# evolbioinfo/pastml

Hardware: AMD Instinct MI355X
Metric: ACR nodes*states*chars/sec (full marginal pass: P(t) + bottom-up + top-down + posteriors) (higher is better)
Workload: dtype f64; 1 GPU; BASELINE config 4 shard: balanced tree, 1048576 tips (2097151 nodes), k=64 states, F81, 32 characters per GPU (32 in total), marginal (BU+TD+posteriors); tips=1048576, nodes=2097151, states=64, chars_per_gpu=32, chars_total=32, substitution_model=F81, collective=local

## Files before the change

pastml_amd/csrc/pml_kernels_f81.h:

```cpp
#pragma once
#include "pml_device.h"
#include "pml_schedule.h"

typedef unsigned char pml_jt;

struct PmlTree {
    int N;
    int n_roots;
    const int* parent;
    const int* first_child;
    const int* n_children;
    const double* dist;
    const int* post_rank;
    const unsigned char* kind;
};

struct PmlCols {
    int k, ks, W;
    int no_wide_lean;
    const u64* masks;
    const u64* masks_init;
    const double* pi;
    const double* active;
};
// ... 1523 lines not shown
template <int G, int R>
__device__ __forceinline__ void bu_f81_super_issue(const LaneCtx<G, R>& L, const SuperRegs& s, SuperLoads<R>& ld) {
#pragma unroll
    for (int j = 0; j < 2; ++j) {
        const UnitRegs u = super_child<G>(s, j, L.g);
        f81_gather_issue<G, R>(L, u, ld.c[j].cl, ld.c[j].tl);
        ld.c[j].own = L.mask[(unsigned)u.n];
    }
    ld.e = L.E[s.fc + (L.g & 1)];
    ld.own = L.mask[(unsigned)s.n];
}

template <int R>
__device__ __forceinline__ void super_loads_arrived(SuperLoads<R>& ld) {
#pragma unroll
    for (int j = 0; j < 2; ++j)
        asm volatile("" : "+v"(ld.c[j].cl.e), "+v"(ld.c[j].cl.mask), "+v"(ld.c[j].tl.e), "+v"(ld.c[j].tl.s),
                          "+v"(ld.c[j].tl.mask), "+v"(ld.c[j].own));
    asm volatile("" : "+v"(ld.e), "+v"(ld.own));
}

template <int G, int R>
__device__ __forceinline__ bool bu_f81_super_unit(const LaneCtx<G, R>& L, const PmlTree& t, const PmlCols& c,
                                                  const PmlState& st, const SuperRegs& s, SuperLoads<R>& ld) {
    super_loads_arrived<R>(ld);
    const u64 kbits = state_bits(c.k);
    bool ones = c.k == G * R;
#pragma unroll
    for (int j = 0; j < 2; ++j) {
        f81_gather_finish<G, R>(L, ld.c[j].cl, ld.c[j].tl);
        ones = ones && (ld.c[j].own & kbits) == kbits && ld.c[j].cl.mask == kbits;
    }
    const bool full = __all(ones);
    BuResult<R> res[2];
#pragma unroll
    for (int j = 0; j < 2; ++j) {
        const UnitRegs u = super_child<G>(s, j, L.g);
        const bool ok = full ? bu_f81_marg_body<G, R, false, true, true>(L, t, c, st, u, ld.c[j], &res[j], false)
                             : bu_f81_marg_body<G, R, false, false, true>(L, t, c, st, u, ld.c[j], &res[j], false);
        if (!ok) return false;
    }
    BuLoads<R> top;
    top.cl.e = ld.e;
    top.cl.s = (L.g & 1) ? res[1].s : res[0].s;
    top.cl.be = (L.g & 1) ? res[1].e : res[0].e;
    top.cl.mask = kbits;
    top.tl.e = top.tl.s = top.tl.a = 0.0;
    top.tl.mask = 0ull;
    top.own = ld.own;
#pragma unroll
    for (int r = 0; r < R; ++r) {
        top.v0[r] = res[0].v[r];
        top.v1[r] = res[1].v[r];
    }
    return bu_f81_marg_body<G, R, true, false>(L, t, c, st, super_own(s), top);
}

template <int G, int R>
__device__ __forceinline__ void bu_f81_super_seq(const LaneCtx<G, R>& L, const PmlTree& t, const PmlCols& c,
                                                 const PmlState& st, const SuperRegs& s) {
    bu_f81_unit_seq<G, R, false>(L, t, c, st, super_child<G>(s, 0, L.g));
    bu_f81_unit_seq<G, R, false>(L, t, c, st, super_child<G>(s, 1, L.g));
    __threadfence();
    bu_f81_unit_seq<G, R, false>(L, t, c, st, super_own(s));
}

template <int G, int R>
__global__ void __launch_bounds__(PML_BLOCK) __attribute__((amdgpu_waves_per_eu(2, 2)))
bu_f81_super_kernel(PmlTree t, PmlCols c, PmlState st, const PmlUnit* __restrict__ units, int n_level) {
    constexpr int UW = 64 / G;
    const int wave = threadIdx.x >> 6;
    const int sub = (threadIdx.x & 63) / G;
    LaneCtx<G, R> L;
    lane_ctx_init<G, R>(L, t, c, st);
    const int stride = gridDim.x * PML_WAVES_PER_BLOCK * UW;
    int idx = (blockIdx.x * PML_WAVES_PER_BLOCK + wave) * UW + sub;
    int base = idx - sub;
    SuperRegs ua = load_super(units, idx < n_level ? idx : 0);
    SuperRegs ub = load_super(units, idx + stride < n_level ? idx + stride : 0);
    SuperLoads<R> la, lb;
    bu_f81_super_issue<G, R>(L, ua, la);
    while (base < n_level) {
        {
            const int i2 = idx + 2 * stride;
            const SuperRegs un = load_super(units, i2 < n_level ? i2 : 0);
            bu_f81_super_issue<G, R>(L, ub, lb);
            if (idx < n_level) {
                if (!bu_f81_super_unit<G, R>(L, t, c, st, ua, la)) bu_f81_super_seq<G, R>(L, t, c, st, ua);
            }
            ua = un;
            idx += stride;
            base += stride;
        }
        if (base >= n_level) break;
        {
            const int i2 = idx + 2 * stride;
            const SuperRegs un = load_super(units, i2 < n_level ? i2 : 0);
            bu_f81_super_issue<G, R>(L, ua, la);
            if (idx < n_level) {
                if (!bu_f81_super_unit<G, R>(L, t, c, st, ub, lb)) bu_f81_super_seq<G, R>(L, t, c, st, ub);
            }
            ub = un;
            idx += stride;
            base += stride;
        }
    }
}

template <int G, int R>
__device__ __forceinline__ void f81_finish_child(const LaneCtx<G, R>& L, const PmlCols& c, const double (&prod)[R],
                                                 i64 pe, int ch, double e, double s_child, i64 bec,
                                                 const double (&v)[R], bool full_mask, const double (&mb)[R],
                                                 double (&tdc)[R], i64& xe, double (&lh)[R], double& lsum, i64& le,
                                                 int slot = -1) {
    const double a = (1.0 - e) * s_child;
    double x[R];
#pragma unroll
    for (int r = 0; r < R; ++r) {
        const double cn = fmax(a + e * v[r], 0x1p-1022);
        x[r] = prod[r] * rcp1(cn);
    }
    xe = pe - bec;
    const double b = (1.0 - e) * pi_dot<G, R>(L, x);
#pragma unroll
    for (int r = 0; r < R; ++r) tdc[r] = b + e * x[r];
    double lhs = 0.0;
    if (full_mask) {
#pragma unroll
        for (int r = 0; r < R; ++r) {
            lh[r] = v[r] * tdc[r] * L.pi_r[r];
            lhs += lh[r];
        }
    } else {
#pragma unroll
        for (int r = 0; r < R; ++r) {
            lh[r] = v[r] * tdc[r] * (L.pi_r[r] * mb[r]);
            lhs += lh[r];
        }
    }
    lhs = group_sum<G>(lhs);
    const int lex = (lhs > 0.0 && !isinf(lhs)) ? exponent_of(lhs) : 0;
    const double inv = rcp1(lhs);
#pragma unroll
    for (int r = 0; r < R; ++r) {
        const double q = lh[r] * inv;
        lh[r] = fma(fma(-lhs, q, lh[r]), inv, q);
    }
    const bool staged = post_row<G, R>(L, c, slot, ch, lh);
    lsum = __builtin_ldexp(lhs, -lex);
    le = xe + bec + lex;
    post_scalars<G, R>(L, staged ? slot : -1, ch, lsum, le);
}

template <int G, int R>
__device__ __forceinline__ void f81_finish_tip_word(const LaneCtx<G, R>& L, const PmlCols& c, const double (&prod)[R],
                                                    i64 pe, double& P, bool& have_P, int tip, u64 word, double e,
                                                    double pis, int slot = -1) {
    if (__popcll(word) == 1) {
        if (!have_P) {
            P = pi_dot<G, R>(L, prod);
            have_P = true;
        }
        double oh[R];
        clean_word_to_vec<G, R>(L, c, word, oh);
        double pick = 0.0;
#pragma unroll
        for (int r = 0; r < R; ++r) pick = fma(oh[r], prod[r], pick);
        const double ps = group_sum<G>(pick);
        const double q = pis * ps;
        double c0 = (1.0 - e) * pis;
        const double c1 = c0 + e;
        if (!(c0 > 0.0)) c0 = 1.0;
        const double r1 = rcp1(c1);
        const double sx = (P - q) * rcp1(c0) + q * r1;
        const double tds = (1.0 - e) * sx + e * (ps * r1);
        const double lhs = tds * pis;
        const bool ok = lhs > 0.0 && !isinf(lhs);
        const int lex = ok ? exponent_of(lhs) : 0;
        if (!ok) {
#pragma unroll
            for (int r = 0; r < R; ++r) oh[r] = __builtin_nan("");
        }
        const bool staged = post_onehot<G, R>(L, c, slot, tip, (int)__builtin_ctzll(word), oh, ok);
        post_scalars<G, R>(L, staged ? slot : -1, tip, __builtin_ldexp(lhs, -lex), pe + lex);
    } else {
        double mt[R], tdt[R], pt[R], lt;
        clean_word_to_vec<G, R>(L, c, word, mt);
        i64 xt, et;
        f81_finish_child<G, R>(L, c, prod, pe, tip, e, pis, 0, mt, false, mt, tdt, xt, pt, lt, et, slot);
    }
}

template <int G, int R>
__device__ __forceinline__ void f81_finish_tip(const LaneCtx<G, R>& L, const PmlCols& c, const double (&prod)[R], i64 pe,
                                               double& P, bool& have_P, int tip, int slot = -1) {
    const double e = L.E[tip];
    const double pis = L.S[tip];
    if (c.W == 1) {
        f81_finish_tip_word<G, R>(L, c, prod, pe, P, have_P, tip, L.mask[(unsigned)tip] & state_bits(c.k), e, pis,
                                  slot);
    } else {
        double mt[R], tdt[R], pt[R], lt;
        node_mask_vec<G, R>(L, c, tip, mt);
        i64 xt, et;
        f81_finish_child<G, R>(L, c, prod, pe, tip, e, pis, 0, mt, false, mt, tdt, xt, pt, lt, et, slot);
    }
}

template <int G, int R>
__device__ __forceinline__ void td_f81_fast_children(const LaneCtx<G, R>& L, const PmlTree& t, const PmlCols& c,
                                                     const PmlState& st, const UnitRegs& u, const double (&prod)[R],
                                                     i64 pe, const ChildLane& cl, const TipLane& tl, double (&vn)[R]);

template <int G, int R>
__device__ __forceinline__ void td_f81_unit_fast(const LaneCtx<G, R>& L, const PmlTree& t, const PmlCols& c,
                                                 const PmlState& st, const UnitRegs& u) {
    const int p = u.n, fc = u.fc;
    double prod[R];
    i64 pe;
    f81_parent_prod<G, R>(L, c, p, prod, pe);
    ChildLane cl;
    TipLane tl;
    f81_gather_issue<G, R>(L, u, cl, tl);
    double vn[R];
    if (unit_code(u.packed, 0) == 1) node_load_vec<G, R>(L, c, L.bu, fc, vn);
    f81_gather_finish<G, R>(L, cl, tl);
    td_f81_fast_children<G, R>(L, t, c, st, u, prod, pe, cl, tl, vn);
}

template <int G, int R>
__device__ __forceinline__ void td_f81_fast_children(const LaneCtx<G, R>& L, const PmlTree& t, const PmlCols& c,
                                                     const PmlState& st, const UnitRegs& u, const double (&prod)[R],
                                                     i64 pe, const ChildLane& cl, const TipLane& tl, double (&vn)[R]) {
    constexpr int GC = Gather<G>::GC;
    const int fc = u.fc;
    const int nc = unit_nc(u.packed);
    double P = 0.0;
    bool have_P = false;
    for (int jx = 0; jx < nc; ++jx) {
        const int src = L.group_base + jx;
        const int ch = fc + jx;
        const int code = unit_code(u.packed, jx);
        const double e = __shfl(cl.e, src, 64);
        const u64 word = __shfl(cl.mask, src, 64);
        double v[R];
        if (code == 1) {
#pragma unroll
            for (int r = 0; r < R; ++r) v[r] = vn[r];
        }
        if (jx + 1 < nc && unit_code(u.packed, jx + 1) == 1) node_load_vec<G, R>(L, c, L.bu, ch + 1, vn);
        if (code == 0) {
            f81_finish_tip_word<G, R>(L, c, prod, pe, P, have_P, ch, word, e, __shfl(cl.s, src, 64));
            continue;
        }
        double mb[R], tdc[R], po[R], ls;
        const bool full = word == state_bits(c.k);
        if (!full) clean_word_to_vec<G, R>(L, c, word, mb);
        i64 xe, le;
        if (code == 1) {
            f81_finish_child<G, R>(L, c, prod, pe, ch, e, __shfl(cl.s, src, 64), __shfl(cl.be, src, 64), v, full, mb,
                                   tdc, xe, po, ls, le);
            if (st.td != nullptr) {
                node_store_vec<G, R>(L, c, L.td, ch, tdc);
                if (L.g == 0) L.te[ch] = xe;
            }
        } else {
            i64 bec;
            const int cfc = __shfl(u.cfc, L.group_base + jx * GC, 64);
            const int cnc = code - 1;
            f81_cherry_from_lanes<G, R>(L, c, cl, tl, jx, cnc, v, bec);
            const double s_child = __shfl(cl.s, src, 64);
            f81_finish_child<G, R>(L, c, prod, pe, ch, e, s_child, bec, v, full, mb, tdc, xe, po, ls, le);
            double prod2[R];
#pragma unroll
            for (int r = 0; r < R; ++r) prod2[r] = po[r] * (ls * L.ipi_r[r]);
            const i64 pe2 = le;
            double P2 = 0.0;
            bool have_P2 = false;
            for (int q = 0; q < cnc; ++q) {
                const int ts = L.group_base + jx * GC + q;
                f81_finish_tip_word<G, R>(L, c, prod2, pe2, P2, have_P2, cfc + q, __shfl(tl.mask, ts, 64),
                                          __shfl(tl.e, ts, 64), __shfl(tl.s, ts, 64));
            }
        }
    }
}

template <int G, int R, int SC0 = PML_SHAPE_ANY, int SC1 = PML_SHAPE_ANY>
__device__ __forceinline__ void td_f81_unit_lean(const LaneCtx<G, R>& L, const PmlTree& t, const PmlCols& c,
                                                 const PmlState& st, const UnitRegs& u) {
    constexpr bool ANY = SC0 == PML_SHAPE_ANY;
    const int p = u.n, fc = u.fc;
    const int nc = ANY ? unit_nc(u.packed) : (SC1 < 0 ? 1 : 2);
    const u64 kbits = state_bits(c.k);
    double po[R];
    node_load_vec<G, R>(L, c, L.post, p, po);
    const double ls = L.lhsum[p];
    const i64 pe = L.lhe[p];
    double ce[2], cs[2], vv[2][R];
    u64 cm[2];
    i64 cbe[2];
    double te[2][2], ts[2][2];
    u64 tm[2][2];
#pragma unroll
    for (int j = 0; j < 2; ++j) {
        const int ch = fc + (j < nc ? j : 0);
        const int code = j < nc ? (ANY ? unit_code(u.packed, j) : (j == 0 ? SC0 : SC1)) : 0;
        ce[j] = L.E[ch];
        cm[j] = L.mask[(unsigned)ch];
        cs[j] = L.S[ch];
        cbe[j] = code == 1 ? L.be[ch] : 0;
        if (code == 1) {
            node_load_vec<G, R>(L, c, L.bu, ch, vv[j]);
        } else {
#pragma unroll
            for (int r = 0; r < R; ++r) vv[j][r] = 0.0;
        }
        const int cfc = j == 0 ? u.cfc : u.cfc1;
#pragma unroll
        for (int q = 0; q < 2; ++q) {
            const bool has = code >= 2 && q < code - 1;
            const int tip = has ? cfc + q : ch;
            te[j][q] = L.E[tip];
            ts[j][q] = has ? L.S[tip] : 0.0;
            tm[j][q] = L.mask[(unsigned)tip];
        }
    }
    double prod[R];
#pragma unroll
    for (int r = 0; r < R; ++r) prod[r] = po[r] * (ls * L.ipi_r[r]);
    double P = 0.0;
    bool have_P = false;
#pragma unroll
    for (int j = 0; j < 2; ++j) {
        if (j < nc) {
            const int ch = fc + j;
            const int code = ANY ? unit_code(u.packed, j) : (j == 0 ? SC0 : SC1);
// ... 310 lines not shown
    const int p = u.n;

    double prod[R];
    i64 pe;
    f81_parent_prod<G, R>(L, c, p, prod, pe);
    double P = 0.0;
    bool have_P = false;
    const int fc = u.fc;
    int nc = unit_nc(u.packed);
    if (nc == 15) nc = t.n_children[p];
    for (int j = 0; j < nc; ++j) {
        const int ch = fc + j;
        const ChildDesc cd = unit_child<G>(t, u, j, ch);
        const int kd = cd.kind;
        const int slot = j < 2 ? j : -1;
        if (kd == PML_KIND_TIP) {
            f81_finish_tip<G, R>(L, c, prod, pe, P, have_P, ch, slot);
            continue;
        }
        const double e = L.E[ch];
        double mb[R], v[R], tdc[R], po[R], ls;
        node_mask_vec<G, R>(L, c, ch, mb);
        i64 xe, le;
        if (kd == PML_KIND_STORED) {
            node_load_vec<G, R>(L, c, L.bu, ch, v);
            f81_finish_child<G, R>(L, c, prod, pe, ch, e, L.S[ch], L.be[ch], v, false, mb, tdc, xe, po, ls, le, slot);
            if (st.td != nullptr) {
                node_store_vec<G, R>(L, c, L.td, ch, tdc);
                if (L.g == 0) L.te[ch] = xe;
            }
        } else {
            i64 bec;
            f81_cherry_vector<G, R>(L, t, c, st, ch, v, bec, false, cd.tips_known, cd.fc2, cd.nc2);
            const double s_child = L.S[ch];
            f81_finish_child<G, R>(L, c, prod, pe, ch, e, s_child, bec, v, false, mb, tdc, xe, po, ls, le, slot);
            double prod2[R];
#pragma unroll
            for (int r = 0; r < R; ++r) prod2[r] = po[r] * (ls * L.ipi_r[r]);
            const i64 pe2 = le;
            double P2 = 0.0;
            bool have_P2 = false;
            const int fc2 = cd.tips_known ? cd.fc2 : t.first_child[ch];
            const int nc2 = cd.tips_known ? cd.nc2 : t.n_children[ch];
            for (int q = 0; q < nc2; ++q)
                f81_finish_tip<G, R>(L, c, prod2, pe2, P2, have_P2, fc2 + q, (j < 2 && q < 2) ? 2 + 2 * j + q : -1);
        }
    }
}

struct TdStage {
    double* rows;
    double* sum;
    i64* exp;
    int* id;
    int* tid;
    int* tst;
};
__host__ __device__ __forceinline__ int td_stage_doubles(int uw, int ks, bool scalars) {
    return uw * 2 * ks + (scalars ? uw * 12 : 0) + uw * 5;
}

template <int G, int R>
__device__ __forceinline__ void td_stage_flush(const LaneCtx<G, R>& L, const PmlCols& c, const TdStage& S, bool tips) {
    typedef double dbl2 __attribute__((ext_vector_type(2)));
    constexpr int UW = 64 / G;
    wave_sync_lds();
    const int lane = threadIdx.x & 63;
    const int ppr = c.ks >> 1;
    for (int p = lane; p < UW * 2 * ppr; p += 64) {
        const int slot = p / ppr, piece = p - slot * ppr;
        const int node = S.id[slot];
        if (node >= 0) {
            const dbl2 v = *reinterpret_cast<const dbl2*>(S.rows + slot * c.ks + 2 * piece);
            __builtin_nontemporal_store(v, reinterpret_cast<dbl2*>(L.post + (size_t)(unsigned)node * c.ks + 2 * piece));
        }
    }
    for (int p = lane; tips && p < UW * 4 * ppr; p += 64) {
        const int slot = p / ppr, piece = p - slot * ppr;
        const int node = S.tid[slot];
        if (node >= 0) {
            const int s = S.tst[slot];
            dbl2 v;
            v.x = s == 2 * piece ? 1.0 : 0.0;
            v.y = s == 2 * piece + 1 ? 1.0 : 0.0;
            __builtin_nontemporal_store(v, reinterpret_cast<dbl2*>(L.post + (size_t)(unsigned)node * c.ks + 2 * piece));
        }
    }
    if (S.sum != nullptr) {
        for (int e = lane; e < UW * 6; e += 64) {
            const int u = e / 6, j = e - u * 6;
            if (j >= 2 && !tips) continue;
            const int node = j < 2 ? S.id[u * 2 + j] : S.tid[u * 4 + j - 2];
            if (node >= 0) {
                L.lhsum[node] = S.sum[e];
                L.lhe[node] = S.exp[e];
            }
        }
    }
    wave_sync_lds();
    for (int e = lane; e < UW * 2; e += 64) S.id[e] = -1;
    for (int e = lane; tips && e < UW * 4; e += 64) S.tid[e] = -1;
    wave_sync_lds();
}

template <int G, int R>
__global__ void __launch_bounds__(PML_BLOCK)
td_f81_kernel(PmlTree t, PmlCols c, PmlState st, const PmlUnit* __restrict__ units, int n_level, int stage) {
    extern __shared__ double td_stage[];
    constexpr int UW = 64 / G;
    const int wave = threadIdx.x >> 6;
    const int sub = (threadIdx.x & 63) / G;
    LaneCtx<G, R> L;
    lane_ctx_init<G, R>(L, t, c, st);
    TdStage S = {nullptr, nullptr, nullptr, nullptr, nullptr, nullptr};
    const bool staged = G <= PML_TD_STAGE_MAX_G && (stage & 1) && (c.ks & 1) == 0;
    if (staged) {
        const bool scalars = (stage & 2) != 0;
        double* base = td_stage + wave * td_stage_doubles(UW, c.ks, scalars);
        S.rows = base;
        base += UW * 2 * c.ks;
        if (scalars) {
            S.sum = base;
            S.exp = reinterpret_cast<i64*>(base + UW * 6);
            base += UW * 12;
        }
        S.id = reinterpret_cast<int*>(base);
        S.tid = S.id + UW * 2;
        S.tst = S.tid + UW * 4;
        L.srow = S.rows + sub * 2 * c.ks;
        L.sid = S.id + sub * 2;
        L.stid = S.tid + sub * 4;
        L.stst = S.tst + sub * 4;
        if (scalars) {
            L.ssum = S.sum + sub * 6;
            L.sexp = S.exp + sub * 6;
        }
        for (int e = threadIdx.x & 63; e < UW * 2; e += 64) S.id[e] = -1;
        for (int e = threadIdx.x & 63; e < UW * 4; e += 64) S.tid[e] = -1;
        wave_sync_lds();
    }
    const int stride = gridDim.x * PML_WAVES_PER_BLOCK * UW;
    int idx = (blockIdx.x * PML_WAVES_PER_BLOCK + wave) * UW + sub;
    UnitRegs cur = load_unit<G>(units, idx < n_level ? idx : 0, L.g);
    for (int base = idx - sub; base < n_level; base += stride) {
        const int nxt_idx = idx + stride;
        const UnitRegs nxt = load_unit<G>(units, nxt_idx < n_level ? nxt_idx : 0, L.g);
        if (idx < n_level) td_f81_unit<G, R, true>(L, t, c, st, cur);
        if (staged) td_stage_flush<G, R>(L, c, S, (stage & 4) != 0);
        cur = nxt;
        idx = nxt_idx;
    }
}

template <int G, int R>
__device__ __forceinline__ void td_f81_super_unit(const LaneCtx<G, R>& L, const PmlTree& t, const PmlCols& c,
                                                  const PmlState& st, const SuperRegs& s, int j) {
    const u64 kbits = state_bits(c.k);
    const int ch = s.fc + j;
    const UnitRegs u = super_child<G>(s, j, L.g);
    double prod[R];
    i64 pe;
    f81_parent_prod<G, R>(L, c, s.n, prod, pe);
    const double e = L.E[ch];
    const double s_child = L.S[ch];
    const i64 bec = L.be[ch];
    BuLoads<R> ld;
    ld.own = L.mask[(unsigned)ch];
    f81_gather_issue<G, R>(L, u, ld.cl, ld.tl);
    f81_gather_finish<G, R>(L, ld.cl, ld.tl);
    ld.own &= kbits;
    const bool all_ones = __all(c.k == G * R && ld.own == kbits && ld.cl.mask == kbits);
    BuResult<R> v;
    CherryKeep<R> ck;
    if (all_ones) bu_f81_marg_body<G, R, false, true, true>(L, t, c, st, u, ld, &v, false, true, &ck);
    else bu_f81_marg_body<G, R, false, false, true>(L, t, c, st, u, ld, &v, false, true, &ck);
    double prod2[R];
    i64 pe2;
    {
        double mb[R], tdc[R], po[R], ls;
        const bool full = ld.own == kbits;
        if (!full) clean_word_to_vec<G, R>(L, c, ld.own, mb);
        i64 xe;
        f81_finish_child<G, R>(L, c, prod, pe, ch, e, s_child, bec, v.v, full, mb, tdc, xe, po, ls, pe2);
        if (st.td != nullptr) {
            node_store_vec<G, R>(L, c, L.td, ch, tdc);
            if (L.g == 0) L.te[ch] = xe;
        }
#pragma unroll
        for (int r = 0; r < R; ++r) prod2[r] = po[r] * (ls * L.ipi_r[r]);
    }
    constexpr int GC = Gather<G>::GC;
#pragma unroll
    for (int jx = 0; jx < 2; ++jx) {
        const int src = L.group_base + jx;
        const int cch = u.fc + jx;
        const double ce = __shfl(ld.cl.e, src, 64);
        const u64 word = __shfl(ld.cl.mask, src, 64);
        double mb[R], tdc[R], po[R], ls;
        const bool full = word == kbits;
        if (!full) clean_word_to_vec<G, R>(L, c, word, mb);
        i64 xe, le;
        const int cfc = __shfl(u.cfc, L.group_base + jx * GC, 64);
        f81_finish_child<G, R>(L, c, prod2, pe2, cch, ce, __shfl(ld.cl.s, src, 64), ck.e[jx], ck.v[jx], full, mb, tdc, xe, po,
                               ls, le);
        double prod3[R];
#pragma unroll
        for (int r = 0; r < R; ++r) prod3[r] = po[r] * (ls * L.ipi_r[r]);
        double P3 = 0.0;
        bool have_P3 = false;
#pragma unroll
        for (int q = 0; q < 2; ++q) {
            const int ts = L.group_base + jx * GC + q;
            f81_finish_tip_word<G, R>(L, c, prod3, le, P3, have_P3, cfc + q, __shfl(ld.tl.mask, ts, 64),
                                      __shfl(ld.tl.e, ts, 64), __shfl(ld.tl.s, ts, 64));
        }
    }
}

template <int G, int R>
__global__ void __launch_bounds__(PML_BLOCK)
td_f81_super_kernel(PmlTree t, PmlCols c, PmlState st, const PmlUnit* __restrict__ units, int n_level) {
    constexpr int UW = 64 / G;
    const int wave = threadIdx.x >> 6;
    const int sub = (threadIdx.x & 63) / G;
    LaneCtx<G, R> L;
    lane_ctx_init<G, R>(L, t, c, st);
    const int n_units = 2 * n_level;
    const int stride = gridDim.x * PML_WAVES_PER_BLOCK * UW;
    int idx = (blockIdx.x * PML_WAVES_PER_BLOCK + wave) * UW + sub;
    SuperRegs cur = load_super(units, idx < n_units ? idx >> 1 : 0);
    for (int base = idx - sub; base < n_units; base += stride) {
        const int nxt_idx = idx + stride;
        const SuperRegs nxt = load_super(units, nxt_idx < n_units ? nxt_idx >> 1 : 0);
        if (idx < n_units) td_f81_super_unit<G, R>(L, t, c, st, cur, idx & 1);
        cur = nxt;
        idx = nxt_idx;
    }
}

struct StackRegs {
    int n, fc, g0, g1;
};

__device__ __forceinline__ StackRegs load_stack(const PmlUnit* __restrict__ units, int idx) {
    const int4 h = *reinterpret_cast<const int4*>(units + idx);
    const int4 f = *reinterpret_cast<const int4*>(units[idx].cfc);
    StackRegs s;
    s.n = h.x;
    s.fc = h.y;
    s.g0 = f.x;
    s.g1 = f.y;
    return s;
}

__device__ __forceinline__ UnitRegs stack_child(const StackRegs& s, int j) {
    UnitRegs u;
    u.n = s.fc + j;
    u.fc = j ? s.g1 : s.g0;
    u.packed = PML_PACKED_TWO_STORED;
    u.cfc = u.cfc1 = u.cfc2 = u.cfc3 = 0;
    return u;
}

template <int G, int R>
__device__ __forceinline__ void stack_child_loads(const LaneCtx<G, R>& L, const PmlCols& c, int node, int first,
                                                  BuLoads<R>& ld) {
    const int ch = first + (L.g & 1);
    ld.cl.e = L.E[ch];
    ld.cl.s = L.S[ch];
    ld.cl.be = L.be[ch];
    ld.cl.mask = 0ull;
    ld.tl.e = ld.tl.s = ld.tl.a = 0.0;
    ld.tl.mask = 0ull;
    ld.own = L.mask[(unsigned)node];
    node_load_vec<G, R>(L, c, L.bu, first, ld.v0);
    node_load_vec<G, R>(L, c, L.bu, first + 1, ld.v1);
}

template <int G, int R>
__device__ __forceinline__ bool bu_f81_stack_unit(const LaneCtx<G, R>& L, const PmlTree& t, const PmlCols& c,
                                                  const PmlState& st, const StackRegs& s) {
    BuLoads<R> ld[2];
#pragma unroll
    for (int j = 0; j < 2; ++j) stack_child_loads<G, R>(L, c, s.fc + j, j ? s.g1 : s.g0, ld[j]);
    const double e_top = L.E[s.fc + (L.g & 1)];
    const u64 own = L.mask[(unsigned)s.n];
    BuResult<R> res[2];
#pragma unroll
    for (int j = 0; j < 2; ++j)
        if (!bu_f81_marg_body<G, R, true, false>(L, t, c, st, stack_child(s, j), ld[j], &res[j], false)) return false;
    BuLoads<R> top;
    top.cl.e = e_top;
    top.cl.s = (L.g & 1) ? res[1].s : res[0].s;
    top.cl.be = (L.g & 1) ? res[1].e : res[0].e;
    top.cl.mask = 0ull;
    top.tl.e = top.tl.s = top.tl.a = 0.0;
    top.tl.mask = 0ull;
    top.own = own;
#pragma unroll
    for (int r = 0; r < R; ++r) {
        top.v0[r] = res[0].v[r];
        top.v1[r] = res[1].v[r];
    }
    UnitRegs un;
    un.n = s.n;
    un.fc = s.fc;
    un.packed = PML_PACKED_TWO_STORED;
    un.cfc = un.cfc1 = un.cfc2 = un.cfc3 = 0;
    return bu_f81_marg_body<G, R, true, false>(L, t, c, st, un, top);
}

template <int G, int R>
__global__ void __launch_bounds__(PML_BLOCK) __attribute__((amdgpu_waves_per_eu(2, 2)))
bu_f81_stack_kernel(PmlTree t, PmlCols c, PmlState st, const PmlUnit* __restrict__ units, int n_level) {
    constexpr int UW = 64 / G;
    const int wave = threadIdx.x >> 6;
    const int sub = (threadIdx.x & 63) / G;
    LaneCtx<G, R> L;
    lane_ctx_init<G, R>(L, t, c, st);
    const int stride = gridDim.x * PML_WAVES_PER_BLOCK * UW;
    int idx = (blockIdx.x * PML_WAVES_PER_BLOCK + wave) * UW + sub;
    StackRegs cur = load_stack(units, idx < n_level ? idx : 0);
    for (int base = idx - sub; base < n_level; base += stride) {
        const int nxt_idx = idx + stride;
        const StackRegs nxt = load_stack(units, nxt_idx < n_level ? nxt_idx : 0);
        if (idx < n_level) {
            if (!bu_f81_stack_unit<G, R>(L, t, c, st, cur)) {
                bu_f81_unit_seq<G, R, false>(L, t, c, st, stack_child(cur, 0));
                bu_f81_unit_seq<G, R, false>(L, t, c, st, stack_child(cur, 1));
                __threadfence();
                UnitRegs un = stack_child(cur, 0);
                un.n = cur.n;
                un.fc = cur.fc;
                bu_f81_unit_seq<G, R, false>(L, t, c, st, un);
            }
        }
        cur = nxt;
        idx = nxt_idx;
    }
}

template <int G, int R>
__device__ __forceinline__ void td_f81_stack_unit(const LaneCtx<G, R>& L, const PmlTree& t, const PmlCols& c,
                                                  const PmlState& st, const StackRegs& s, int j) {
    const u64 kbits = state_bits(c.k);
    const int ch = s.fc + j;
    const int first = j ? s.g1 : s.g0;
    double prod[R];
    i64 pe;
    f81_parent_prod<G, R>(L, c, s.n, prod, pe);
    const double e = L.E[ch];
    const double s_child = L.S[ch];
    const i64 bec = L.be[ch];
    BuLoads<R> ld;
    stack_child_loads<G, R>(L, c, ch, first, ld);
    const u64 gmask = L.mask[(unsigned)(first + (L.g & 1))] & kbits;
    ld.own &= kbits;
    BuResult<R> v;
    double g0v[R], g1v[R];
#pragma unroll
    for (int r = 0; r < R; ++r) {
        g0v[r] = ld.v0[r];
        g1v[r] = ld.v1[r];
    }
    bu_f81_marg_body<G, R, true, false>(L, t, c, st, stack_child(s, j), ld, &v, false, true);
    double prod2[R];
    i64 pe2;
    {
        double mb[R], tdc[R], po[R], ls;
        const bool full = ld.own == kbits;
        if (!full) clean_word_to_vec<G, R>(L, c, ld.own, mb);
        i64 xe;
        f81_finish_child<G, R>(L, c, prod, pe, ch, e, s_child, bec, v.v, full, mb, tdc, xe, po, ls, pe2);
        if (st.td != nullptr) {
            node_store_vec<G, R>(L, c, L.td, ch, tdc);
            if (L.g == 0) L.te[ch] = xe;
        }
#pragma unroll
        for (int r = 0; r < R; ++r) prod2[r] = po[r] * (ls * L.ipi_r[r]);
    }
#pragma unroll
    for (int jx = 0; jx < 2; ++jx) {
        const int src = L.group_base + jx;
        const u64 word = __shfl(gmask, src, 64);
        double mb[R], tdc[R], po[R], ls;
        const bool full = word == kbits;
        if (!full) clean_word_to_vec<G, R>(L, c, word, mb);
// ... 269 lines not shown
```

pastml_amd/csrc/pml_launch_f81_super.hip:

```cpp
#include "pml_launch.h"

template <int G, int R>
static void launch_super_f81(pml_ctx* ctx, bool bottom_up) {
    const PmlTree t = tree_of(ctx, true);
    const PmlCols c = cols_of(ctx, bottom_up);
    const PmlState st = state_of(ctx);
    const int upb = PML_WAVES_PER_BLOCK * (64 / G);
    dim3 grid(grid_for(ctx, bottom_up ? ctx->sup.n : 2 * ctx->sup.n, upb, ctx->C, bottom_up), ctx->C), block(PML_BLOCK);
    if (bottom_up)
        hipLaunchKernelGGL((bu_f81_super_kernel<G, R>), grid, block, 0, ctx->stream, t, c, st, ctx->sup.d_units, ctx->sup.n);
    else
        hipLaunchKernelGGL((td_f81_super_kernel<G, R>), grid, block, 0, ctx->stream, t, c, st, ctx->sup.d_units, ctx->sup.n);
}

template <int G, int R>
static void launch_stack_f81(pml_ctx* ctx, bool bottom_up, int a, int n) {
    const PmlTree t = tree_of(ctx, true);
    const PmlCols c = cols_of(ctx, bottom_up);
    const PmlState st = state_of(ctx);
    const int upb = PML_WAVES_PER_BLOCK * (64 / G);
    dim3 grid(grid_for(ctx, bottom_up ? n : 2 * n, upb, ctx->C), ctx->C), block(PML_BLOCK);
    if (bottom_up)
        hipLaunchKernelGGL((bu_f81_stack_kernel<G, R>), grid, block, 0, ctx->stream, t, c, st, ctx->sup.d_stack_bu + a, n);
    else
        hipLaunchKernelGGL((td_f81_stack_kernel<G, R>), grid, block, 0, ctx->stream, t, c, st, ctx->sup.d_stack_td + a, n);
}

int dispatch_super_f81(pml_ctx* ctx, bool bottom_up) {
    if (ctx->sup.n <= 0) return PML_OK;
    int g, r;
    super_shape(ctx, bottom_up, g, r);
#define X(G_, R_)                                   \
    if (g == G_ && r == R_) {                       \
        launch_super_f81<G_, R_>(ctx, bottom_up);   \
        HIP_TRY(hipGetLastError());                 \
        return PML_OK;                              \
    }
    PML_SUPER_CASES(X)
#undef X
    return fail(PML_ERR_UNSUPPORTED, "no two-level F81 kernel for G=%d R=%d", g, r);
}

int dispatch_stack_f81(pml_ctx* ctx, bool bottom_up, int level) {
    const std::vector<int>& off = bottom_up ? ctx->sup.stack_bu_offsets : ctx->sup.stack_td_offsets;
    if (ctx->sup.n_stack == 0 || level + 1 >= (int)off.size()) return PML_OK;
    const int a = off[level], n = off[level + 1] - a;
    if (n <= 0) return PML_OK;
    int g, r;
    super_shape(ctx, bottom_up, g, r);
#define X(G_, R_)                                         \
    if (g == G_ && r == R_) {                             \
        launch_stack_f81<G_, R_>(ctx, bottom_up, a, n);   \
        HIP_TRY(hipGetLastError());                       \
        return PML_OK;                                    \
    }
    PML_SUPER_CASES(X)
#undef X
    return fail(PML_ERR_UNSUPPORTED, "no stacked F81 kernel for G=%d R=%d", g, r);
}
```

pastml_amd/csrc/pml_schedule.h:

```cpp
#pragma once
#include <cstdlib>
#include <string>
#include <vector>

#define PML_KIND_TIP 0
#define PML_KIND_CHERRY 1
#define PML_KIND_STORED 2

struct __attribute__((aligned(32))) PmlUnit {
    int n, fc, packed, pad;
    int cfc[4];
};

#define PML_PACKED_TWO_STORED ((1 << 11) | (1 << 8) | (3 << 4) | 2)

#define PML_TUNABLES(X)                                                                                              \
    X(GRID_CAP, 0, 0) X(SMALL_MANY_NODES, 0, 0) X(BLOCK_MAX_WORK, 0, 0)    \
    X(NO_MFMA, 1, 0) X(NO_EIGEN_FUSED, 1, 0) X(NO_HKY_FUSED, 1, 0)      \
    X(BLOCK_THREADS, 0, 0) X(EIG_BLOCKS, 0, 0) X(NO_EIGEN_GEMM, 1, 0) X(NO_EIGEN_JOINT_VALU, 1, 0) X(EIGJ_BLOCKS, 0, 0) \
    X(EIGJ_TIP_BLOCKS, 0, 0) X(EIGJ_ONE_TIPS_KERNEL, 1, 0) X(EIGJ_TIER_THIN, 0, 1) X(EIGJ_TIER_DEPTH, 0, 1)            \
    X(NO_EIGJ_TIERS, 1, 1) X(NO_BT_TIERS, 1, 1) X(NO_SHAPE_SORT, 1, 1) X(NO_SUPER, 1, 1) X(SUPER_MIN, 0, 1)            \
    X(STACK_MIN, 0, 1) X(NO_STACK, 1, 1) X(DEBUG, 1, 0) X(BLOCK_NODES, 0, 1) X(BLOCK_MAX_STORED, 0, 1)                 \
    X(BLOCK_HEIGHT_CAP, 0, 1) X(SMALL_MAX_NODES, 0, 1) X(F81_R, 0, 1) X(F81_TD_R, 0, 1) X(NO_GRAPH, 1, 1)              \
    X(NARROW_UNITS, 0, 0) X(NO_EIGG_TIERS, 1, 0) X(NO_SPIN_WAIT, 1, 0)   \
    X(PIJ_STAGE_ROWS, 0, 0) X(PIJ_BLOCKS, 0, 0) X(NO_HEIGHT_ORDER, 1, 1) X(NO_TD_TAIL, 1, 0) X(NO_PIJ_VALU, 1, 0) X(PIJ_VALU, 1, 0) X(NO_PIJ_WIDE, 1, 0) X(NO_EIGJ_PIPE, 1, 0) \
    X(THIN_UNITS, 0, 1) X(THIN_BYTES, 0, 1) X(THIN_BLOCK_NODES, 0, 1) X(NO_THIN, 1, 0) X(NO_THIN_WIDE, 1, 0) X(BU_WIDE, 0, 1) X(SORT_LEVELS, 0, 1) X(NO_WIDE_LEAN, 1, 0) X(SHAPE_ORDER, 0, 1) \
    X(PARS_MAX_COLS, 0, 0) X(PARS_THIN, 0, 0) X(COMPRESS_MAX_COLS, 0, 0) X(COMPRESS_PLAIN_ATOMICS, 1, 0) \
    X(PIJ_WINDOW, 0, 0) X(NO_KEEP_TIP_ROWS, 1, 0)
enum PmlTunable {
#define X(name, flag, tree) T_##name,
    PML_TUNABLES(X)
#undef X
    T_COUNT
};
static const char* const kTunableName[T_COUNT] = {
#define X(name, flag, tree) #name,
    PML_TUNABLES(X)
#undef X
};
static const bool kTunableFlag[T_COUNT] = {
#define X(name, flag, tree) flag != 0,
    PML_TUNABLES(X)
#undef X
};
static const bool kTunableTree[T_COUNT] = {
#define X(name, flag, tree) tree != 0,
    PML_TUNABLES(X)
#undef X
};
struct PmlTune {
    long long val[T_COUNT];
    bool has[T_COUNT];
    PmlTune() {
        for (int i = 0; i < T_COUNT; ++i) {
            const std::string var = std::string("PASTML_HIP_") + kTunableName[i];
            const char* e = getenv(var.c_str());
            has[i] = e != nullptr;
            val[i] = e ? atoll(e) : 0;
        }
    }
    bool on(int i) const { return has[i]; }
    long long get(int i, long long dflt) const { return has[i] ? val[i] : dflt; }
};

struct PmlBlockSchedule {
    bool ok = false;
    int n_blocks = 0;
    long long steps = 0;
    PmlUnit *d_bu_units = nullptr, *d_td_units = nullptr;
    int *d_bu_start = nullptr, *d_bu_levels = nullptr, *d_bu_lv = nullptr;
    int *d_td_start = nullptr, *d_td_levels = nullptr, *d_td_lv = nullptr;
    PmlUnit *d_top_bu_units = nullptr, *d_top_td_units = nullptr;
    int *d_top_bu_offsets = nullptr, *d_top_td_offsets = nullptr;
    std::vector<int> top_bu_offsets, top_td_offsets;
    std::vector<char> top_bu_vec;
};
struct PmlThinSchedule {
    bool ok = false;
    int floor_level = 0;
    int top_level = 0;
    struct Tier { int first_block, n_blocks; };
    std::vector<Tier> tiers;
    PmlUnit* d_units = nullptr;
    int *d_start = nullptr, *d_levels = nullptr, *d_lv = nullptr;
};
struct PmlDeepSchedule {
    bool ok = false;
    int first_depth = 0, n_blocks = 0;
    PmlUnit* d_units = nullptr;
    int *d_start = nullptr, *d_levels = nullptr, *d_lv = nullptr;
};
struct PmlSuperSchedule {
    bool ok = false;
    int n = 0;
    PmlUnit* d_units = nullptr;
    PmlUnit* d_child_units = nullptr;
    PmlUnit *d_bu_units_r = nullptr, *d_td_units_r = nullptr;
    PmlUnit *d_bu_units_rs = nullptr, *d_td_units_rs = nullptr;
    int n_child_units = 0;
    int n_stack = 0;
    PmlUnit *d_stack_bu = nullptr, *d_stack_td = nullptr, *d_stack_children = nullptr;
    std::vector<int> stack_bu_offsets, stack_td_offsets;
    int *d_bu_offsets_r = nullptr, *d_td_offsets_r = nullptr;
    std::vector<int> bu_offsets_r, td_offsets_r;
    std::vector<char> bu_level_vec_r;
};
struct PmlEigenTiers {
    bool ok = false;
    int first_level = 0;
    int top_level = 0;
    struct Tier { int first_block, n_blocks, depth; };
    std::vector<Tier> tiers;
    PmlUnit* d_units = nullptr;
    int *d_lv = nullptr, *d_start = nullptr;
    int* d_nodes = nullptr;
    int widest = 0;
};
struct PmlBacktraceTiers {
    bool ok = false;
    int first_depth = 0;
    struct Tier { int first_block, n_blocks, depth; };
    std::vector<Tier> tiers;
    int *d_nodes = nullptr, *d_lv = nullptr, *d_start = nullptr;
};

struct PmlTreeArrays {
    int n_nodes, n_roots, n_bu_levels, n_td_levels;
    const int *parent, *first_child, *n_children, *bu_offsets, *bu_order, *td_offsets, *td_parent_offsets, *td_parents,
        *post_rank;
    const double* dist;
};

struct PmlNumbering {
    std::vector<int> old_of_new, new_of_old;
    std::vector<int> parent, first_child, n_children, bu_order, td_parents, post_rank;
    std::vector<double> dist;
};

struct PmlForest {
    bool fuse = true;
    int N = 0, n_roots = 0, n_internal = 0;
    std::vector<int> parent, first_child, n_children;
    std::vector<int> bu_offsets, td_offsets, td_parent_offsets;
    std::vector<unsigned char> kind;
    std::vector<int> fh;
    std::vector<int> order_f;
    std::vector<int> bu_offsets_f;
    std::vector<int> tdp;
    std::vector<int> td_parent_offsets_f;
    bool shape_ordered = false;
    bool polytomies = false;
    bool balanced_parts = false;
    int max_h() const { return (int)bu_offsets_f.size() - 1; }
    int n_stored() const { return bu_offsets_f.empty() ? 0 : bu_offsets_f.back(); }
};

struct PmlLevelTable {
    std::vector<int> list, start, levels, lv;
    template <class F>
    void add_runs(const int* mem, size_t count, F level) {
        start.push_back((int)lv.size());
        int nl = 0;
        for (size_t q = 0; q < count; ++q) {
            if (q == 0 || level(mem[q]) != level(mem[q - 1])) {
                lv.push_back((int)list.size());
                ++nl;
            }
            list.push_back(mem[q]);
        }
        lv.push_back((int)list.size());
        levels.push_back(nl);
    }
    template <class F>
    void add_cells(const int* mem, size_t count, F level, int first, int n) {
        start.push_back((int)lv.size());
        size_t q = 0;
        for (int d = 0; d < n; ++d) {
            lv.push_back((int)list.size());
            for (; q < count && level(mem[q]) == first + d; ++q) list.push_back(mem[q]);
        }
        lv.push_back((int)list.size());
// ... 114 lines not shown
```

Before: 543.7 billion node*state*char/s.

## Process super-unit tip posteriors in parallel lanes via LDS row lookup

```diff
diff --git a/pastml_amd/csrc/pml_kernels_f81.h b/pastml_amd/csrc/pml_kernels_f81.h
--- a/pastml_amd/csrc/pml_kernels_f81.h
+++ b/pastml_amd/csrc/pml_kernels_f81.h
@@ -1699,6 +1699,22 @@
     post_scalars<G, R>(L, staged ? slot : -1, ch, lsum, le);
 }
 
+__device__ __forceinline__ void f81_tip_closed_form(double P, double ps, double e, double pis, i64 pe, double& lhs,
+                                                    bool& ok, double& lsum, i64& le) {
+    const double q = pis * ps;
+    double c0 = (1.0 - e) * pis;
+    const double c1 = c0 + e;
+    if (!(c0 > 0.0)) c0 = 1.0;
+    const double r1 = rcp1(c1);
+    const double sx = (P - q) * rcp1(c0) + q * r1;
+    const double tds = (1.0 - e) * sx + e * (ps * r1);
+    lhs = tds * pis;
+    ok = lhs > 0.0 && !isinf(lhs);
+    const int lex = ok ? exponent_of(lhs) : 0;
+    lsum = __builtin_ldexp(lhs, -lex);
+    le = pe + lex;
+}
+
 template <int G, int R>
 __device__ __forceinline__ void f81_finish_tip_word(const LaneCtx<G, R>& L, const PmlCols& c, const double (&prod)[R],
                                                     i64 pe, double& P, bool& have_P, int tip, u64 word, double e,
@@ -1714,22 +1730,16 @@
 #pragma unroll
         for (int r = 0; r < R; ++r) pick = fma(oh[r], prod[r], pick);
         const double ps = group_sum<G>(pick);
-        const double q = pis * ps;
-        double c0 = (1.0 - e) * pis;
-        const double c1 = c0 + e;
-        if (!(c0 > 0.0)) c0 = 1.0;
-        const double r1 = rcp1(c1);
-        const double sx = (P - q) * rcp1(c0) + q * r1;
-        const double tds = (1.0 - e) * sx + e * (ps * r1);
-        const double lhs = tds * pis;
-        const bool ok = lhs > 0.0 && !isinf(lhs);
-        const int lex = ok ? exponent_of(lhs) : 0;
+        double lhs, lsum;
+        bool ok;
+        i64 le;
+        f81_tip_closed_form(P, ps, e, pis, pe, lhs, ok, lsum, le);
         if (!ok) {
 #pragma unroll
             for (int r = 0; r < R; ++r) oh[r] = __builtin_nan("");
         }
         const bool staged = post_onehot<G, R>(L, c, slot, tip, (int)__builtin_ctzll(word), oh, ok);
-        post_scalars<G, R>(L, staged ? slot : -1, tip, __builtin_ldexp(lhs, -lex), pe + lex);
+        post_scalars<G, R>(L, staged ? slot : -1, tip, lsum, le);
     } else {
         double mt[R], tdt[R], pt[R], lt;
         clean_word_to_vec<G, R>(L, c, word, mt);
@@ -2346,9 +2356,24 @@
     }
 }
 
-template <int G, int R>
+
+template <int G, int R>
+__device__ __forceinline__ void td_f81_super_tips(const LaneCtx<G, R>& L, const PmlCols& c, const double (&prod3)[R],
+                                                  i64 le, int cfc, const TipLane& tl, int jx) {
+    constexpr int GC = Gather<G>::GC;
+    double P3 = 0.0;
+    bool have_P3 = false;
+#pragma unroll
+    for (int q = 0; q < 2; ++q) {
+        const int ts = L.group_base + jx * GC + q;
+        f81_finish_tip_word<G, R>(L, c, prod3, le, P3, have_P3, cfc + q, __shfl(tl.mask, ts, 64), __shfl(tl.e, ts, 64),
+                                  __shfl(tl.s, ts, 64));
+    }
+}
+
+template <int G, int R, bool LANES>
 __device__ __forceinline__ void td_f81_super_unit(const LaneCtx<G, R>& L, const PmlTree& t, const PmlCols& c,
-                                                  const PmlState& st, const SuperRegs& s, int j) {
+                                                  const PmlState& st, const SuperRegs& s, int j, double* ps_row) {
     const u64 kbits = state_bits(c.k);
     const int ch = s.fc + j;
     const UnitRegs u = super_child<G>(s, j, L.g);
@@ -2384,6 +2409,11 @@
         for (int r = 0; r < R; ++r) prod2[r] = po[r] * (ls * L.ipi_r[r]);
     }
     constexpr int GC = Gather<G>::GC;
+    const bool tip_lane = (L.g & ~(GC | 1)) == 0;
+    const int tjx = (L.g / GC) & 1;
+    bool lanes = LANES && c.W == 1 && !group_any<G>(tip_lane && __popcll(ld.tl.mask) != 1);
+    double prod3[2][R], P3[2], ps = 0.0;
+    i64 le3[2];
 #pragma unroll
     for (int jx = 0; jx < 2; ++jx) {
         const int src = L.group_base + jx;
@@ -2393,30 +2423,65 @@
         double mb[R], tdc[R], po[R], ls;
         const bool full = word == kbits;
         if (!full) clean_word_to_vec<G, R>(L, c, word, mb);
-        i64 xe, le;
-        const int cfc = __shfl(u.cfc, L.group_base + jx * GC, 64);
+        i64 xe;
         f81_finish_child<G, R>(L, c, prod2, pe2, cch, ce, __shfl(ld.cl.s, src, 64), ck.e[jx], ck.v[jx], full, mb, tdc, xe, po,
-                               ls, le);
-        double prod3[R];
-#pragma unroll
-        for (int r = 0; r < R; ++r) prod3[r] = po[r] * (ls * L.ipi_r[r]);
-        double P3 = 0.0;
-        bool have_P3 = false;
-#pragma unroll
-        for (int q = 0; q < 2; ++q) {
-            const int ts = L.group_base + jx * GC + q;
-            f81_finish_tip_word<G, R>(L, c, prod3, le, P3, have_P3, cfc + q, __shfl(ld.tl.mask, ts, 64),
-                                      __shfl(ld.tl.e, ts, 64), __shfl(ld.tl.s, ts, 64));
-        }
-    }
-}
-
-template <int G, int R>
+                               ls, le3[jx]);
+#pragma unroll
+        for (int r = 0; r < R; ++r) prod3[jx][r] = po[r] * (ls * L.ipi_r[r]);
+        if (!lanes) {
+            td_f81_super_tips<G, R>(L, c, prod3[jx], le3[jx], __shfl(u.cfc, L.group_base + jx * GC, 64), ld.tl, jx);
+            continue;
+        }
+        P3[jx] = pi_dot<G, R>(L, prod3[jx]);
+#pragma unroll
+        for (int r = 0; r < R; r += 2) {
+            double2 t2;
+            t2.x = prod3[jx][r];
+            t2.y = prod3[jx][r + 1];
+            *reinterpret_cast<double2*>(ps_row + L.st(r)) = t2;
+        }
+        wave_sync_lds();
+        if (tip_lane && tjx == jx) ps = ps_row[__builtin_ctzll(ld.tl.mask)];
+        wave_sync_lds();
+    }
+    if (!lanes) return;
+    double lhs, lsum;
+    bool ok;
+    i64 le;
+    f81_tip_closed_form(tjx ? P3[1] : P3[0], ps, ld.tl.e, ld.tl.s, tjx ? le3[1] : le3[0], lhs, ok, lsum, le);
+    lanes = !isinf(P3[0]) && !isnan(P3[0]) && !isinf(P3[1]) && !isnan(P3[1]) && !group_any<G>(tip_lane && !ok);
+    if (!lanes) {
+#pragma unroll
+        for (int jx = 0; jx < 2; ++jx)
+            td_f81_super_tips<G, R>(L, c, prod3[jx], le3[jx], __shfl(u.cfc, L.group_base + jx * GC, 64), ld.tl, jx);
+        return;
+    }
+    if (tip_lane) {
+        const int tip = u.cfc + (L.g & 1);
+        L.lhsum[tip] = lsum;
+        L.lhe[tip] = le;
+    }
+    if (!L.implicit_tips) {
+        const int ts = (int)__builtin_ctzll(ld.tl.mask | (1ull << 63));
+#pragma unroll
+        for (int q = 0; q < 4; ++q) {
+            const int sq = __shfl(ts, L.group_base + (q >> 1) * GC + (q & 1), 64);
+            double oh[R];
+#pragma unroll
+            for (int r = 0; r < R; ++r) oh[r] = L.st(r) == sq ? 1.0 : 0.0;
+            node_store_vec_nt<G, R>(L, c, L.post, s.t0 + 4 * j + q, oh);
+        }
+    }
+}
+
+template <int G, int R, bool LANES>
 __global__ void __launch_bounds__(PML_BLOCK)
 td_f81_super_kernel(PmlTree t, PmlCols c, PmlState st, const PmlUnit* __restrict__ units, int n_level) {
     constexpr int UW = 64 / G;
     const int wave = threadIdx.x >> 6;
     const int sub = (threadIdx.x & 63) / G;
+    __shared__ __attribute__((aligned(16))) double tip_rows[LANES ? PML_BLOCK * R : 2];
+    double* const ps_row = LANES ? tip_rows + (wave * UW + sub) * (G * R) : nullptr;
     LaneCtx<G, R> L;
     lane_ctx_init<G, R>(L, t, c, st);
     const int n_units = 2 * n_level;
@@ -2426,7 +2491,7 @@
     for (int base = idx - sub; base < n_units; base += stride) {
         const int nxt_idx = idx + stride;
         const SuperRegs nxt = load_super(units, nxt_idx < n_units ? nxt_idx >> 1 : 0);
-        if (idx < n_units) td_f81_super_unit<G, R>(L, t, c, st, cur, idx & 1);
+        if (idx < n_units) td_f81_super_unit<G, R, LANES>(L, t, c, st, cur, idx & 1, ps_row);
         cur = nxt;
         idx = nxt_idx;
     }
diff --git a/pastml_amd/csrc/pml_launch_f81_super.hip b/pastml_amd/csrc/pml_launch_f81_super.hip
--- a/pastml_amd/csrc/pml_launch_f81_super.hip
+++ b/pastml_amd/csrc/pml_launch_f81_super.hip
@@ -9,8 +9,10 @@
     dim3 grid(grid_for(ctx, bottom_up ? ctx->sup.n : 2 * ctx->sup.n, upb, ctx->C, bottom_up), ctx->C), block(PML_BLOCK);
     if (bottom_up)
         hipLaunchKernelGGL((bu_f81_super_kernel<G, R>), grid, block, 0, ctx->stream, t, c, st, ctx->sup.d_units, ctx->sup.n);
+    else if (ctx->tune.on(T_NO_TIP_LANES))
+        hipLaunchKernelGGL((td_f81_super_kernel<G, R, false>), grid, block, 0, ctx->stream, t, c, st, ctx->sup.d_units, ctx->sup.n);
     else
-        hipLaunchKernelGGL((td_f81_super_kernel<G, R>), grid, block, 0, ctx->stream, t, c, st, ctx->sup.d_units, ctx->sup.n);
+        hipLaunchKernelGGL((td_f81_super_kernel<G, R, true>), grid, block, 0, ctx->stream, t, c, st, ctx->sup.d_units, ctx->sup.n);
 }
 
 template <int G, int R>
diff --git a/pastml_amd/csrc/pml_schedule.h b/pastml_amd/csrc/pml_schedule.h
--- a/pastml_amd/csrc/pml_schedule.h
+++ b/pastml_amd/csrc/pml_schedule.h
@@ -26,7 +26,7 @@
     X(PIJ_STAGE_ROWS, 0, 0) X(PIJ_BLOCKS, 0, 0) X(NO_HEIGHT_ORDER, 1, 1) X(NO_TD_TAIL, 1, 0) X(NO_PIJ_VALU, 1, 0) X(PIJ_VALU, 1, 0) X(NO_PIJ_WIDE, 1, 0) X(NO_EIGJ_PIPE, 1, 0) \
     X(THIN_UNITS, 0, 1) X(THIN_BYTES, 0, 1) X(THIN_BLOCK_NODES, 0, 1) X(NO_THIN, 1, 0) X(NO_THIN_WIDE, 1, 0) X(BU_WIDE, 0, 1) X(SORT_LEVELS, 0, 1) X(NO_WIDE_LEAN, 1, 0) X(SHAPE_ORDER, 0, 1) \
     X(PARS_MAX_COLS, 0, 0) X(PARS_THIN, 0, 0) X(COMPRESS_MAX_COLS, 0, 0) X(COMPRESS_PLAIN_ATOMICS, 1, 0) \
-    X(PIJ_WINDOW, 0, 0) X(NO_KEEP_TIP_ROWS, 1, 0)
+    X(PIJ_WINDOW, 0, 0) X(NO_KEEP_TIP_ROWS, 1, 0) X(NO_TIP_LANES, 1, 0)
 enum PmlTunable {
 #define X(name, flag, tree) T_##name,
     PML_TUNABLES(X)
```

Measured after the change: 572.9 billion node*state*char/s, median of 6. 5.4% higher.
